# evapachetti/3d_vit_ensemble

Hardware: NVIDIA B200
Metric: ensemble volumes/sec (inference, fwd+bwd train) at 1/2/4/8 B200 vs CPU ref (higher is better)
Workload: dtype bf16

## Files before the change

3d_vit_ensemble_b200/csrc/api.cu:

```cuda
#include <stdarg.h>

#include "common.cuh"
#include "kernels.cuh"
#include "tc.cuh"

namespace vit3d {

static thread_local char g_err[512] = "";
static unsigned long long g_launches = 0;
void count_launch() { __atomic_fetch_add(&g_launches, 1ull, __ATOMIC_RELAXED); }

void set_error(const char* fmt, ...) {
  va_list ap;
  va_start(ap, fmt);
  vsnprintf(g_err, sizeof(g_err), fmt, ap);
  va_end(ap);
}
int cuda_fail(cudaError_t e, const char* what, const char* file, int line) {
  set_error("CUDA error %d (%s) at %s:%d: %s", (int)e, cudaGetErrorString(e), file, line, what);
  return VIT3D_ERR_CUDA;
}
int sm_count() {
  static thread_local int cached_dev = -1, cached = 0;
  int dev = 0;
  if (cudaGetDevice(&dev) != cudaSuccess) return 148;
  if (dev != cached_dev) {
    cudaDeviceProp p;
    if (cudaGetDeviceProperties(&p, dev) != cudaSuccess) return 148;
    cached = p.multiProcessorCount;
    cached_dev = dev;
  }
  return cached;
}

static int g_tuning[VIT3D_TUNE_COUNT] = {
    0,
    0,
    0,
    0,
    0,
    0,
    1,
    1,
    0,
    1,
    0,
    0,
    0,
    0,
    0,
};
constexpr unsigned kLiveTuningKeys =
    1u << VIT3D_TUNE_ATTN_THREADS | 1u << VIT3D_TUNE_MLP_PAIR | 1u << VIT3D_TUNE_WGRAD_RED | 1u << VIT3D_TUNE_ATTN_BWD |
    1u << VIT3D_TUNE_RES_PAIR | 1u << VIT3D_TUNE_ATTN_TF32 | 1u << VIT3D_TUNE_PATCH_TALL | 1u << VIT3D_TUNE_PATCH_CLUSTER |
    1u << VIT3D_TUNE_ATTN_FWD_UNIT;
static bool tuning_key_live(int key) { return key >= 0 && key < VIT3D_TUNE_COUNT && ((kLiveTuningKeys >> key) & 1u); }
int tuning(int key) {
  return (key >= 0 && key < VIT3D_TUNE_COUNT) ? __atomic_load_n(&g_tuning[key], __ATOMIC_RELAXED) : 0;
}

static inline int act_f32(int prec) { return prec != VIT3D_PREC_BF16; }

}

using namespace vit3d;

extern "C" {

int vit3d_version(void) { return VIT3D_VERSION; }
const char* vit3d_last_error(void) { return g_err; }

int vit3d_device_info(int* sms, int* cc) {
  int dev = 0;
  V3_CUDA(cudaGetDevice(&dev));
  cudaDeviceProp p;
  V3_CUDA(cudaGetDeviceProperties(&p, dev));
  if (sms) *sms = p.multiProcessorCount;
  if (cc) *cc = p.major * 10 + p.minor;
  return VIT3D_OK;
}
int vit3d_set_tuning(int key, int value) {
  V3_REQUIRE(tuning_key_live(key), "set_tuning: unknown or retired key %d", key);
  __atomic_store_n(&g_tuning[key], value, __ATOMIC_RELAXED);
  return VIT3D_OK;
}
int vit3d_get_tuning(int key) {
  V3_REQUIRE(tuning_key_live(key), "get_tuning: unknown or retired key %d", key);
  return tuning(key);
}
unsigned long long vit3d_launch_count(void) { return __atomic_load_n(&g_launches, __ATOMIC_RELAXED); }
int vit3d_act_bytes(int prec) { return prec == VIT3D_PREC_BF16 ? 2 : 4; }
int vit3d_tc_supported(int prec, int M, int N, int K) { return tc_linear_supported(prec, M, N, K) ? 1 : 0; }

int vit3d_patch_gather(const float* x, float* patches, int B, int X, int Y, int Z, int p0, int p1, int p2,
                       vit3d_stream_t stream) {
  V3_REQUIRE(B >= 0 && p0 > 0 && p1 > 0 && p2 > 0 && X >= p0 && Y >= p1 && Z >= p2, "patch_gather: bad shape");
  if (B == 0) return VIT3D_OK;
  V3_REQUIRE(x && patches, "patch_gather: null pointer");
  return launch_patch_gather(x, patches, 1, B, X, Y, Z, p0, p1, p2, as_stream(stream));
}

size_t vit3d_patch_embed_ws_bytes(int B, int X, int Y, int Z, int p0, int p1, int p2, int H, int prec) {
  (void)prec;
  const size_t P = (size_t)(X / p0) * (Y / p1) * (Z / p2);
  const size_t Kp = (size_t)p0 * p1 * p2;
  return sizeof(float) * ((size_t)B * P * Kp + (size_t)B * P * H) + 256;
}

int vit3d_patch_embed_fwd(const float* x, const float* w, const float* bias, const float* cls, const float* pos,
                          float* tokens, int B, int X, int Y, int Z, int p0, int p1, int p2, int H, int prec, void* ws,
                          size_t ws_bytes, vit3d_stream_t stream) {
  V3_REQUIRE(x && w && bias && cls && pos && tokens, "patch_embed_fwd: null pointer");
  V3_REQUIRE(B >= 0 && p0 > 0 && p1 > 0 && p2 > 0 && X >= p0 && Y >= p1 && Z >= p2 && H > 0, "patch_embed_fwd: bad shape");
  cudaStream_t st = as_stream(stream);
  const int P = (X / p0) * (Y / p1) * (Z / p2), Kp = p0 * p1 * p2, S = P + 1;
  if (B == 0) return VIT3D_OK;
  if (prec == VIT3D_PREC_BF16 && tc_patch_embed_supported(B, X, Y, Z, p0, p1, p2, H)) {
    int rc = tc_patch_embed_fwd(x, w, bias, pos, tokens, B, X, Y, Z, p0, p1, p2, H, st);
    if (rc != VIT3D_OK) return rc;
    return launch_cls_rows(cls, pos, tokens, B, S, H, st);
  }
  V3_REQUIRE(ws && ws_bytes >= vit3d_patch_embed_ws_bytes(B, X, Y, Z, p0, p1, p2, H, prec), "patch_embed_fwd: workspace too small");
  if (prec == VIT3D_PREC_TF32 && tc_patch_embed_supported(B, X, Y, Z, p0, p1, p2, H) &&
      (size_t)B * X * Y * Z * sizeof(float) <= ws_bytes) {
    float* xr = reinterpret_cast<float*>(ws);
    int rc = launch_round_tf32(x, xr, (long long)B * X * Y * Z, st);
    if (rc != VIT3D_OK) return rc;
    rc = tc_patch_embed_fwd(xr, w, bias, pos, tokens, B, X, Y, Z, p0, p1, p2, H, st);
    if (rc != VIT3D_OK) return rc;
    return launch_cls_rows(cls, pos, tokens, B, S, H, st);
  }
  float* patches = reinterpret_cast<float*>(ws);
  int rc = launch_patch_gather(x, patches, 1, B, X, Y, Z, p0, p1, p2, st);
  if (rc != VIT3D_OK) return rc;
  SgemmArgs g;
  g.A = patches; g.sa_m = Kp; g.sa_k = 1;
  g.B = w; g.sb_k = 1; g.sb_n = Kp;
  g.C = tokens; g.ldc = H;
  g.bias = bias; g.rowadd = pos; g.row_group = P;
  g.M = B * P; g.N = H; g.K = Kp;
  rc = launch_sgemm(g, st);
  if (rc != VIT3D_OK) return rc;
  return launch_cls_rows(cls, pos, tokens, B, S, H, st);
}

int vit3d_patch_embed_bwd(const float* x, const float* dtokens, float* dw, float* dbias, float* dcls, float* dpos, int B,
                          int X, int Y, int Z, int p0, int p1, int p2, int H, int prec, void* ws, size_t ws_bytes,
                          vit3d_stream_t stream) {
  V3_REQUIRE(x && dtokens && dw && dbias && dcls && dpos, "patch_embed_bwd: null pointer");
  V3_REQUIRE(ws && ws_bytes >= vit3d_patch_embed_ws_bytes(B, X, Y, Z, p0, p1, p2, H, prec), "patch_embed_bwd: workspace too small");
  cudaStream_t st = as_stream(stream);
  const int P = (X / p0) * (Y / p1) * (Z / p2), Kp = p0 * p1 * p2, S = P + 1;
  if (B == 0) return VIT3D_OK;
  int rc;
  if (prec == VIT3D_PREC_BF16 && tc_wgrad_supported(prec, B * P, H, Kp)) {
    __nv_bfloat16* patches = reinterpret_cast<__nv_bfloat16*>(ws);
    __nv_bfloat16* dYb = patches + (size_t)B * P * Kp;
    rc = launch_patch_gather(x, patches, 0, B, X, Y, Z, p0, p1, p2, st);
    if (rc != VIT3D_OK) return rc;
    rc = launch_gather_patch_rows(dtokens, dYb, 0, B, P, H, st);
    if (rc != VIT3D_OK) return rc;
    rc = tc_gemm_wgrad(dYb, patches, dw, H, Kp, B * P, st);
    if (rc != VIT3D_OK) return rc;
    rc = launch_colsum(dYb, 0, dbias, B * P, H, st);
    if (rc != VIT3D_OK) return rc;
    return launch_embed_param_grads(dtokens, dpos, dcls, B, S, H, st);
  }
  float* patches = reinterpret_cast<float*>(ws);
  float* dY = patches + (size_t)B * P * Kp;
  rc = launch_patch_gather(x, patches, 1, B, X, Y, Z, p0, p1, p2, st);
  if (rc != VIT3D_OK) return rc;
  rc = launch_gather_patch_rows(dtokens, dY, 1, B, P, H, st);
  if (rc != VIT3D_OK) return rc;
  SgemmArgs g;
  g.A = dY; g.sa_m = 1; g.sa_k = H;
  g.B = patches; g.sb_k = Kp; g.sb_n = 1;
  g.C = dw; g.ldc = Kp; g.accumulate = 1;
  g.M = H; g.N = Kp; g.K = B * P;
  g.splitk = pick_splitk(g.M, g.N, g.K);
  rc = launch_sgemm(g, st);
  if (rc != VIT3D_OK) return rc;
  rc = launch_colsum(dY, 1, dbias, B * P, H, st);
  if (rc != VIT3D_OK) return rc;
  return launch_embed_param_grads(dtokens, dpos, dcls, B, S, H, st);
}

int vit3d_patch_embed_dgrad(const float* dtokens, const float* w, const void* w_t_lp, float* dx, int B, int X, int Y, int Z,
                            int p0, int p1, int p2, int H, int prec, void* ws, size_t ws_bytes, vit3d_stream_t stream) {
  V3_REQUIRE(B >= 0 && p0 > 0 && p1 > 0 && p2 > 0 && X >= p0 && Y >= p1 && Z >= p2 && H > 0, "patch_embed_dgrad: bad shape");
  if (B == 0) return VIT3D_OK;
  V3_REQUIRE(dtokens && w && dx, "patch_embed_dgrad: null pointer");
  V3_REQUIRE(ws && ws_bytes >= vit3d_patch_embed_ws_bytes(B, X, Y, Z, p0, p1, p2, H, prec), "patch_embed_dgrad: workspace too small");
  cudaStream_t st = as_stream(stream);
  const int P = (X / p0) * (Y / p1) * (Z / p2), Kp = p0 * p1 * p2, S = P + 1;
  int rc;
  const bool aligned = ((reinterpret_cast<uintptr_t>(dtokens) | reinterpret_cast<uintptr_t>(dx) |
                         reinterpret_cast<uintptr_t>(w_t_lp)) & 15) == 0;
  if (prec != VIT3D_PREC_FP32 && w_t_lp && aligned && tc_patch_dgrad_supported(B, X, Y, Z, p0, p1, p2, H)) {
    const float* a = dtokens;
    if (prec == VIT3D_PREC_TF32) {
      V3_REQUIRE((size_t)B * S * H * sizeof(float) <= ws_bytes, "patch_embed_dgrad: workspace too small");
      float* dr = reinterpret_cast<float*>(ws);
      rc = launch_round_tf32(dtokens, dr, (long long)B * S * H, st);
      if (rc != VIT3D_OK) return rc;
      a = dr;
    }
    return tc_patch_dgrad(a, reinterpret_cast<const float*>(w_t_lp), dx, B, X, Y, Z, p0, p1, p2, H, st);
  }
  float* patches = reinterpret_cast<float*>(ws);
  float* dY = patches + (size_t)B * P * Kp;
  rc = launch_gather_patch_rows(dtokens, dY, 1, B, P, H, st);
  if (rc != VIT3D_OK) return rc;
  SgemmArgs g;
  g.A = dY; g.sa_m = H; g.sa_k = 1;
  g.B = w; g.sb_k = Kp; g.sb_n = 1;
  g.C = patches; g.ldc = Kp;
  g.M = B * P; g.N = Kp; g.K = H;
  rc = launch_sgemm(g, st);
  if (rc != VIT3D_OK) return rc;
  return launch_patch_scatter(patches, dx, B, X, Y, Z, p0, p1, p2, st);
}

int vit3d_ln_fwd(const float* x, const float* gamma, const float* beta, void* y, int y_bf16, float* mean, float* rstd,
                 int M, int H, float eps, vit3d_stream_t stream) {
  V3_REQUIRE(x && gamma && beta && y, "ln_fwd: null pointer");
  V3_REQUIRE(M >= 0 && H > 0, "ln_fwd: bad shape");
  return launch_ln_fwd(x, gamma, beta, y, y_bf16, mean, rstd, M, H, eps, as_stream(stream));
}
int vit3d_ln_bwd(const float* dy, const float* x, const float* mean, const float* rstd, const float* gamma,
                 const float* dres, float* dx, float* dgamma, float* dbeta, int M, int H, vit3d_stream_t stream) {
  V3_REQUIRE(dy && x && mean && rstd && gamma && dx && dgamma && dbeta, "ln_bwd: null pointer");
  V3_REQUIRE(M >= 0 && H > 0 && H <= 8192, "ln_bwd: bad shape");
  return launch_ln_bwd(dy, x, mean, rstd, gamma, dres, dx, dgamma, dbeta, M, H, as_stream(stream));
}

int vit3d_linear_fwd(const void* x, int ldx, int x_f32, const float* w, const void* w_lp, const float* bias,
                     const float* residual, void* y, int y_f32, void* pre, int act, int M, int N, int K, int prec,
                     vit3d_stream_t stream) {
  V3_REQUIRE(x && w && y, "linear_fwd: null pointer");
  V3_REQUIRE(M >= 0 && N > 0 && K > 0 && ldx >= K, "linear_fwd: bad shape M=%d N=%d K=%d ldx=%d", M, N, K, ldx);
  V3_REQUIRE(!(pre && residual), "linear_fwd: pre-activation output and residual are exclusive");
  cudaStream_t st = as_stream(stream);
  if (M == 0) return VIT3D_OK;
  const int xf = x_f32 || act_f32(prec);
  const int yf = y_f32 || residual != nullptr || act_f32(prec);
  if (prec != VIT3D_PREC_FP32 && tc_linear_supported(prec, M, N, K) && (prec == VIT3D_PREC_TF32 ? xf : !xf) &&
      (prec == VIT3D_PREC_TF32 || w_lp) && ldx == K) {
    TcLinear t;
    t.x = x; t.w = w_lp ? w_lp : (const void*)w; t.bias = bias; t.residual = residual;
    t.y = y; t.y_f32 = yf; t.pre = pre; t.act = act; t.M = M; t.N = N; t.K = K; t.prec = prec;
    return tc_linear_fwd(t, st);
  }
  if (N <= 8 && xf && yf && !residual && !pre && act == VIT3D_ACT_NONE)
    return launch_rowdot(reinterpret_cast<const float*>(x), ldx, w, bias, reinterpret_cast<float*>(y), M, N, K, st);
  SgemmArgs g;
  g.A = x; g.sa_m = ldx; g.sa_k = 1; g.a_f32 = xf;
  g.B = w; g.sb_k = 1; g.sb_n = K; g.b_f32 = 1;
  g.C = y; g.ldc = N; g.c_f32 = yf;
  g.bias = bias; g.residual = residual; g.ldr = N; g.pre = pre; g.act = act;
  g.M = M; g.N = N; g.K = K;
  return launch_sgemm(g, st);
}

int vit3d_linear_ln_supported(int M, int N, int K) { return tc_linear_ln_supported(VIT3D_PREC_BF16, M, N, K) ? 1 : 0; }

int vit3d_linear_ln_fwd(const void* x, const void* w_lp, const float* bias, const float* residual, float* y,
                        const float* gamma, const float* beta, float eps, void* ln_out, float* mean, float* rstd, int M,
                        int N, int K, vit3d_stream_t stream) {
  V3_REQUIRE(x && w_lp && y && gamma && beta && ln_out, "linear_ln_fwd: null pointer");
  V3_REQUIRE(M >= 0 && N > 0 && K > 0, "linear_ln_fwd: bad shape M=%d N=%d K=%d", M, N, K);
  if (M == 0) return VIT3D_OK;
  if (!tc_linear_ln_supported(VIT3D_PREC_BF16, M, N, K))
    V3_UNSUPPORTED("linear_ln_fwd: needs BF16 mode shapes with N == 256 (got M=%d N=%d K=%d)", M, N, K);
  TcLinear t;
  t.x = x; t.w = w_lp; t.bias = bias; t.residual = residual; t.y = y; t.y_f32 = 1; t.M = M; t.N = N; t.K = K;
  t.prec = VIT3D_PREC_BF16;
  t.ln_gamma = gamma; t.ln_beta = beta; t.ln_out = ln_out; t.ln_mean = mean; t.ln_rstd = rstd; t.ln_eps = eps;
  return tc_linear_fwd(t, as_stream(stream));
}

int vit3d_linear_bwd(const void* dy, int dy_f32, const void* x, int ldx, int x_f32, const float* w, const void* w_t_lp,
                     void* dx, int lddx, int dx_f32, float* dw, float* db, int M, int N, int K, int prec,
                     vit3d_stream_t stream) {
  V3_REQUIRE(dy && w, "linear_bwd: null pointer");
  V3_REQUIRE(M >= 0 && N > 0 && K > 0, "linear_bwd: bad shape");
  V3_REQUIRE(!dw || x, "linear_bwd: dw needs x");
  cudaStream_t st = as_stream(stream);
  if (M == 0) return VIT3D_OK;
  const int dyf = dy_f32 || act_f32(prec);
  const int xf = x_f32 || act_f32(prec);
  const int dxf = dx_f32 || act_f32(prec);
  int rc;
  if (dx) {
    if (prec == VIT3D_PREC_BF16 && !dyf && w_t_lp && (lddx <= 0 || lddx == K) && tc_linear_supported(prec, M, K, N)) {
      TcLinear t;
      t.x = dy; t.w = w_t_lp; t.y = dx; t.y_f32 = dxf; t.M = M; t.N = K; t.K = N; t.prec = prec;
      rc = tc_linear_fwd(t, st);
    } else {
      SgemmArgs g;
      g.A = dy; g.sa_m = N; g.sa_k = 1; g.a_f32 = dyf;
      g.B = w; g.sb_k = K; g.sb_n = 1; g.b_f32 = 1;
      g.C = dx; g.ldc = lddx > 0 ? lddx : K; g.c_f32 = dxf;
      g.M = M; g.N = K; g.K = N;
      rc = launch_sgemm(g, st);
    }
    if (rc != VIT3D_OK) return rc;
  }
  if (dw) {
    if (!dyf && !xf && ldx == K && tc_wgrad_supported(prec, M, N, K)) {
      rc = tc_gemm_wgrad(dy, x, dw, N, K, M, st);
    } else {
      SgemmArgs g;
      g.A = dy; g.sa_m = 1; g.sa_k = N; g.a_f32 = dyf;
      g.B = x; g.sb_k = ldx; g.sb_n = 1; g.b_f32 = xf;
      g.C = dw; g.ldc = K; g.c_f32 = 1; g.accumulate = 1;
      g.M = N; g.N = K; g.K = M;
      g.splitk = pick_splitk(g.M, g.N, g.K);
      rc = launch_sgemm(g, st);
    }
    if (rc != VIT3D_OK) return rc;
  }
  if (db) {
    rc = launch_colsum(dy, dyf, db, M, N, st);
    if (rc != VIT3D_OK) return rc;
  }
  return VIT3D_OK;
}

int vit3d_mlp_fwd(const void* xn, const void* w1_lp, const float* b1, const void* w2_lp, const float* b2,
                  const float* residual, float* out, int M, int H, int d, vit3d_stream_t stream) {
  V3_REQUIRE(xn && w1_lp && b1 && w2_lp && b2 && residual && out, "mlp_fwd: null pointer");
  V3_REQUIRE(M >= 0 && H > 0 && d > 0, "mlp_fwd: bad shape");
  if (M == 0) return VIT3D_OK;
  return tc_mlp2_fwd(xn, w1_lp, b1, w2_lp, b2, residual, out, nullptr, nullptr, 0.f, nullptr, 0, M, H, d, as_stream(stream));
}
int vit3d_mlp_supported(int M, int H, int d) { return tc_mlp2_supported(M, H, d) ? 1 : 0; }

int vit3d_mlp_ln_supported(int M, int H, int d) { return tc_mlp2_supported(M, H, d) ? 1 : 0; }
int vit3d_mlp_ln_fwd(const void* xn, const void* w1_lp, const float* b1, const void* w2_h, const float* b2,
                     const float* residual, float* out, const float* gamma, const float* beta, float eps, void* ln_out,
                     int M, int H, int d, vit3d_stream_t stream) {
  V3_REQUIRE(xn && w1_lp && b1 && w2_h && b2 && residual && out && gamma && beta && ln_out, "mlp_ln_fwd: null pointer");
  V3_REQUIRE(M >= 0 && H > 0 && d > 0, "mlp_ln_fwd: bad shape");
  if (M == 0) return VIT3D_OK;
  return tc_mlp2_fwd(xn, w1_lp, b1, w2_h, b2, residual, out, gamma, beta, eps, ln_out, 0, M, H, d, as_stream(stream));
}
int vit3d_mlp_lnf_fwd(const void* xn, const void* w1_lp, const float* b1, const void* w2_h, const float* b2,
                      const float* residual, const float* gamma, const float* beta, float eps, float* ln_out, int M, int H,
                      int d, vit3d_stream_t stream) {
  V3_REQUIRE(xn && w1_lp && b1 && w2_h && b2 && residual && gamma && beta && ln_out, "mlp_lnf_fwd: null pointer");
  V3_REQUIRE(M >= 0 && H > 0 && d > 0, "mlp_lnf_fwd: bad shape");
  if (M == 0) return VIT3D_OK;
  return tc_mlp2_fwd(xn, w1_lp, b1, w2_h, b2, residual, nullptr, gamma, beta, eps, ln_out, 1, M, H, d, as_stream(stream));
}

int vit3d_attn_fwd(const void* qkv, void* ctx, float* probs, int B, int S, int heads, int D, int prec,
                   vit3d_stream_t stream) {
  V3_REQUIRE(qkv && ctx, "attn_fwd: null pointer");
  V3_REQUIRE(B >= 0 && S > 0 && heads > 0 && D > 0, "attn_fwd: bad shape");
  cudaStream_t st = as_stream(stream);
  if (prec == VIT3D_PREC_BF16 && tc_attn_supported(S, heads, D)) return tc_attn_fwd(qkv, ctx, probs, S, B, S, heads, D, st);
  if (prec == VIT3D_PREC_TF32 && tc_attn_supported(S, heads, D) && tuning(VIT3D_TUNE_ATTN_TF32) != 0)
    return tc_attn_fwd_tf32(reinterpret_cast<const float*>(qkv), reinterpret_cast<float*>(ctx), probs, S, B, S, heads, D, 1, st);
  return launch_attn_fwd_generic(qkv, act_f32(prec), ctx, probs, B, S, heads, D, prec == VIT3D_PREC_TF32, st);
}
int vit3d_attn_fwd_padded(const void* qkv, void* ctx, float* probs, int probs_ld, int B, int S, int heads, int D,
                          vit3d_stream_t stream) {
  V3_REQUIRE(qkv && ctx && probs, "attn_fwd_padded: null pointer");
  V3_REQUIRE(B >= 0 && S > 0 && heads > 0 && D > 0 && probs_ld >= S, "attn_fwd_padded: bad shape");
  if (!tc_attn_supported(S, heads, D)) V3_UNSUPPORTED("attn_fwd_padded: unsupported shape S=%d heads=%d D=%d", S, heads, D);
  return tc_attn_fwd(qkv, ctx, probs, probs_ld, B, S, heads, D, as_stream(stream));
}
int vit3d_attn_padded_supported(int S, int heads, int D) { return tc_attn_supported(S, heads, D) ? 1 : 0; }
int vit3d_attn_bwd(const void* dctx, const void* qkv, void* dqkv, int B, int S, int heads, int D, int prec,
                   vit3d_stream_t stream) {
  V3_REQUIRE(dctx && qkv && dqkv, "attn_bwd: null pointer");
  V3_REQUIRE(B >= 0 && S > 0 && heads > 0 && D > 0, "attn_bwd: bad shape");
  if (prec == VIT3D_PREC_BF16 && tc_attn_supported(S, heads, D)) return tc_attn_bwd(dctx, qkv, dqkv, nullptr, nullptr, nullptr, B, S, heads, D, as_stream(stream));
  return launch_attn_bwd_generic(dctx, qkv, act_f32(prec), dqkv, B, S, heads, D, as_stream(stream));
}

int vit3d_gelu_fwd(const void* h, void* a, long long n, int prec, vit3d_stream_t stream) {
  V3_REQUIRE(h && a && n >= 0, "gelu_fwd: bad argument");
  return launch_gelu_fwd(h, a, n, act_f32(prec), as_stream(stream));
}
int vit3d_gelu_bwd(const void* da, const void* h, void* dh, long long n, int prec, vit3d_stream_t stream) {
  V3_REQUIRE(da && h && dh && n >= 0, "gelu_bwd: bad argument");
  return launch_gelu_bwd(da, h, dh, n, act_f32(prec), as_stream(stream));
}
int vit3d_gelu_dropout_bwd(const void* da, const void* h, void* dh, long long n, int prec, float p,
                           unsigned long long seed, unsigned site, unsigned step, const unsigned* step_dev,
                           vit3d_stream_t stream) {
  V3_REQUIRE(da && h && dh && n >= 0 && p >= 0.f && p < 1.f, "gelu_dropout_bwd: bad argument");
  if (!gelu_dropout_bwd_supported(da, h, dh, n, act_f32(prec)))
    V3_UNSUPPORTED("gelu_dropout_bwd: needs bf16 activations, 16-byte aligned buffers and n %% 8 == 0");
  return launch_gelu_dropout_bwd(da, h, dh, n, p, seed, site, step, step_dev, as_stream(stream));
}
int vit3d_dropout(const void* x, const void* residual, void* y, long long n, int is_f32, float p,
                  unsigned long long seed, unsigned site, unsigned step, const unsigned* step_dev,
                  vit3d_stream_t stream) {
  V3_REQUIRE(x && y && n >= 0 && p >= 0.f && p < 1.f, "dropout: bad argument");
  return launch_dropout(x, residual, y, n, is_f32, p, seed, site, step, step_dev, as_stream(stream));
}
int vit3d_dropout_mask(unsigned char* mask, long long n, float p, unsigned long long seed, unsigned site, unsigned step,
                       vit3d_stream_t stream) {
  V3_REQUIRE(mask && n >= 0 && p >= 0.f && p < 1.f, "dropout_mask: bad argument");
  return launch_dropout_mask(mask, n, p, seed, site, step, as_stream(stream));
}
int vit3d_dropout_masked(const void* x, const unsigned char* mask, const void* residual, void* y, long long n,
                         int is_f32, float p, vit3d_stream_t stream) {
  V3_REQUIRE(x && mask && y && n >= 0 && p >= 0.f && p < 1.f, "dropout_masked: bad argument");
  return launch_dropout_masked(x, mask, residual, y, n, is_f32, p, as_stream(stream));
}
int vit3d_cast_f32_to_bf16(const float* x, void* y, long long n, vit3d_stream_t stream) {
  V3_REQUIRE(x && y && n >= 0, "cast: bad argument");
  return launch_cast(x, 1, y, 0, n, as_stream(stream));
}
int vit3d_transpose_f32_to_bf16(const float* x, void* y, int rows, int cols, vit3d_stream_t stream) {
  V3_REQUIRE(x && y && rows >= 0 && cols >= 0, "transpose: bad argument");
  return launch_transpose_cast(x, y, rows, cols, as_stream(stream));
}
int vit3d_u8_to_f32(const unsigned char* x, float* y, long long n, float mean, vit3d_stream_t stream) {
  V3_REQUIRE(x && y && n >= 0, "u8_to_f32: bad argument");
  return launch_u8_to_f32(x, y, n, mean, as_stream(stream));
}
int vit3d_round_tf32(const float* x, float* y, long long n, vit3d_stream_t stream) {
  V3_REQUIRE(x && y && n >= 0, "round_tf32: bad argument");
  return launch_round_tf32(x, y, n, as_stream(stream));
}
int vit3d_cast_f32_to_f16(const float* x, void* y, long long n, vit3d_stream_t stream) {
// ... 170 lines not shown
```

3d_vit_ensemble_b200/csrc/tc.cuh:

```cuda
#pragma once
#include "common.cuh"

namespace vit3d {

struct TcLinear {
  const void* x = nullptr;
  const void* w = nullptr;
  const float* bias = nullptr;
  const float* residual = nullptr;
  void* y = nullptr;
  int y_f32 = 0;
  void* pre = nullptr;
  int act = 0;
  int M = 0, N = 0, K = 0, prec = 0;
  const float* ln_gamma = nullptr;
  const float* ln_beta = nullptr;
  void* ln_out = nullptr;
  float* ln_mean = nullptr;
  float* ln_rstd = nullptr;
  float ln_eps = 1e-6f;
  const uint32_t* drop_bits = nullptr;
  float drop_scale = 1.f;
  int store_dact = 0;
};
bool tc_linear_ln_supported(int prec, int M, int N, int K);
bool tc_res_supported(int M, int N, int K, bool ln);
int tc_gemm_res(const TcLinear& t, cudaStream_t st);

bool tc_linear_supported(int prec, int M, int N, int K);
int tc_linear_fwd(const TcLinear& t, cudaStream_t st);

bool tc_wgrad_supported(int prec, int M, int N, int K);
int tc_gemm_wgrad(const void* dy, const void* x, float* dw, int N, int K, int M, cudaStream_t st);
void tc_wgrad_plan(int N, int K, int M, int* bn, int* splits, int* tiles);
int tc_gemm_wgrad_partial(const void* dy, const void* x, float* ws, int N, int K, int M, cudaStream_t st);
int tc_gemm_wgrad_seg(const void* dy, const void* x, float* dw0, float* dw1, float* dw2, int seg_rows, int N, int K, int M,
                      cudaStream_t st);

bool tc_patch_embed_supported(int B, int X, int Y, int Z, int p0, int p1, int p2, int H);
int tc_patch_embed_fwd(const float* x, const float* w, const float* bias, const float* pos, float* tokens, int B, int X,
                       int Y, int Z, int p0, int p1, int p2, int H, cudaStream_t st);
bool tc_patch_dgrad_supported(int B, int X, int Y, int Z, int p0, int p1, int p2, int H);
int tc_patch_dgrad(const float* dtokens, const float* w_t, float* dx, int B, int X, int Y, int Z, int p0, int p1, int p2,
                   int H, cudaStream_t st);

bool tc_mlp3_supported(int M, int H, int d);
int tc_mlp3(const void* xn, const void* w1, const float* b1, const void* w2_h, const float* b2, const float* residual,
            float* y, const float* gamma, const float* beta, float eps, void* ln_out, int ln_f32, int M, int H, int d,
            cudaStream_t st);
bool tc_mlp2_supported(int M, int H, int d);
int tc_mlp2_fwd(const void* xn, const void* w1, const float* b1, const void* w2_h, const float* b2, const float* residual,
                float* y, const float* gamma, const float* beta, float eps, void* ln_out, int ln_f32, int M, int H, int d,
                cudaStream_t st);

bool tc_mlp_bwd_supported(int M, int H, int d);
int tc_mlp_bwd(const void* gy, const void* w2_t, const void* w1_t, const void* dact, void* dh, float* dxn, float* db1, int M,
               int H, int d, cudaStream_t st);

bool tc_attn_supported(int S, int heads, int D);
int tc_attn_fwd(const void* qkv, void* ctx, float* probs, int probs_ld, int B, int S, int heads, int D, cudaStream_t st);
int tc_attn_fwd_tf32(const float* qkv, float* ctx, float* probs, int probs_ld, int B, int S, int heads, int D, int round_out,
                     cudaStream_t st);
int tc_attn_bwd(const void* dctx, const void* qkv, void* dqkv, float* db_q, float* db_k, float* db_v, int B, int S,
                int heads, int D, cudaStream_t st);

}
```

include/vit3d.h:

```cpp
#ifndef VIT3D_H_
#define VIT3D_H_

#include <stddef.h>
#include <stdint.h>

#if defined(__GNUC__)
#pragma GCC visibility push(default)
#endif
#ifdef __cplusplus
extern "C" {
#endif

#define VIT3D_VERSION 100

typedef void* vit3d_stream_t;

enum { VIT3D_OK = 0, VIT3D_ERR_INVALID = -1, VIT3D_ERR_UNSUPPORTED = -2, VIT3D_ERR_CUDA = -3 };
enum { VIT3D_PREC_FP32 = 0, VIT3D_PREC_TF32 = 1, VIT3D_PREC_BF16 = 2 };
enum { VIT3D_ACT_NONE = 0, VIT3D_ACT_GELU = 1 };

int vit3d_version(void);
const char* vit3d_last_error(void);
int vit3d_device_info(int* sm_count, int* cc);
unsigned long long vit3d_launch_count(void);
enum { VIT3D_TUNE_ATTN_THREADS = 1, VIT3D_TUNE_MLP_PAIR = 5, VIT3D_TUNE_WGRAD_RED = 6, VIT3D_TUNE_ATTN_BWD = 7,
       VIT3D_TUNE_RES_PAIR = 8, VIT3D_TUNE_ATTN_TF32 = 9, VIT3D_TUNE_PATCH_TALL = 11, VIT3D_TUNE_PATCH_CLUSTER = 12,
       VIT3D_TUNE_ATTN_FWD_UNIT = 14, VIT3D_TUNE_COUNT = 15 };
int vit3d_set_tuning(int key, int value);
int vit3d_get_tuning(int key);
int vit3d_act_bytes(int prec);
int vit3d_tc_supported(int prec, int M, int N, int K);


int vit3d_patch_gather(const float* x, float* patches, int B, int X, int Y, int Z, int p0, int p1, int p2,
                       vit3d_stream_t stream);
size_t vit3d_patch_embed_ws_bytes(int B, int X, int Y, int Z, int p0, int p1, int p2, int H, int prec);
int vit3d_patch_embed_fwd(const float* x, const float* w, const float* bias, const float* cls, const float* pos,
                          float* tokens, int B, int X, int Y, int Z, int p0, int p1, int p2, int H, int prec,
                          void* ws, size_t ws_bytes, vit3d_stream_t stream);
int vit3d_patch_embed_bwd(const float* x, const float* dtokens, float* dw, float* dbias, float* dcls, float* dpos,
                          int B, int X, int Y, int Z, int p0, int p1, int p2, int H, int prec,
                          void* ws, size_t ws_bytes, vit3d_stream_t stream);
int vit3d_patch_embed_dgrad(const float* dtokens, const float* w, const void* w_t_lp, float* dx,
                            int B, int X, int Y, int Z, int p0, int p1, int p2, int H, int prec,
                            void* ws, size_t ws_bytes, vit3d_stream_t stream);

int vit3d_ln_fwd(const float* x, const float* gamma, const float* beta, void* y, int y_bf16, float* mean,
                 float* rstd, int M, int H, float eps, vit3d_stream_t stream);
int vit3d_ln_bwd(const float* dy, const float* x, const float* mean, const float* rstd, const float* gamma,
                 const float* dres, float* dx, float* dgamma, float* dbeta, int M, int H, vit3d_stream_t stream);

int vit3d_linear_fwd(const void* x, int ldx, int x_f32, const float* w, const void* w_lp, const float* bias,
                     const float* residual, void* y, int y_f32, void* pre, int act, int M, int N, int K, int prec,
                     vit3d_stream_t stream);
int vit3d_linear_ln_fwd(const void* x, const void* w_lp, const float* bias, const float* residual, float* y,
                        const float* gamma, const float* beta, float eps, void* ln_out, float* mean, float* rstd, int M,
                        int N, int K, vit3d_stream_t stream);
int vit3d_linear_ln_supported(int M, int N, int K);
int vit3d_linear_bwd(const void* dy, int dy_f32, const void* x, int ldx, int x_f32, const float* w, const void* w_t_lp,
                     void* dx, int lddx, int dx_f32, float* dw, float* db, int M, int N, int K, int prec,
                     vit3d_stream_t stream);

int vit3d_mlp_fwd(const void* xn, const void* w1_lp, const float* b1, const void* w2_h, const float* b2,
                  const float* residual, float* out, int M, int H, int d, vit3d_stream_t stream);
int vit3d_mlp_supported(int M, int H, int d);
int vit3d_mlp_ln_fwd(const void* xn, const void* w1_lp, const float* b1, const void* w2_h, const float* b2,
                     const float* residual, float* out, const float* gamma, const float* beta, float eps, void* ln_out,
                     int M, int H, int d, vit3d_stream_t stream);
int vit3d_mlp_ln_supported(int M, int H, int d);
int vit3d_mlp_lnf_fwd(const void* xn, const void* w1_lp, const float* b1, const void* w2_h, const float* b2,
                      const float* residual, const float* gamma, const float* beta, float eps, float* ln_out, int M, int H,
                      int d, vit3d_stream_t stream);

int vit3d_attn_fwd(const void* qkv, void* ctx, float* probs, int B, int S, int heads, int D, int prec,
                   vit3d_stream_t stream);
int vit3d_attn_fwd_padded(const void* qkv, void* ctx, float* probs, int probs_ld, int B, int S, int heads, int D,
                          vit3d_stream_t stream);
int vit3d_attn_padded_supported(int S, int heads, int D);
int vit3d_attn_bwd(const void* dctx, const void* qkv, void* dqkv, int B, int S, int heads, int D, int prec,
                   vit3d_stream_t stream);

int vit3d_gelu_fwd(const void* h, void* a, long long n, int prec, vit3d_stream_t stream);
int vit3d_gelu_bwd(const void* da, const void* h, void* dh, long long n, int prec, vit3d_stream_t stream);
int vit3d_gelu_dropout_bwd(const void* da, const void* h, void* dh, long long n, int prec, float p,
                           unsigned long long seed, unsigned site, unsigned step, const unsigned* step_dev,
                           vit3d_stream_t stream);
int vit3d_dropout(const void* x, const void* residual, void* y, long long n, int is_f32, float p,
                  unsigned long long seed, unsigned site, unsigned step, const unsigned* step_dev,
                  vit3d_stream_t stream);
int vit3d_dropout_mask(unsigned char* mask, long long n, float p, unsigned long long seed, unsigned site,
                       unsigned step, vit3d_stream_t stream);
int vit3d_dropout_masked(const void* x, const unsigned char* mask, const void* residual, void* y, long long n,
                         int is_f32, float p, vit3d_stream_t stream);
int vit3d_cast_f32_to_bf16(const float* x, void* y, long long n, vit3d_stream_t stream);
int vit3d_cast_bf16_to_f32(const void* x, float* y, long long n, vit3d_stream_t stream);
int vit3d_cast_f32_to_f16(const float* x, void* y, long long n, vit3d_stream_t stream);
int vit3d_u8_to_f32(const unsigned char* x, float* y, long long n, float mean, vit3d_stream_t stream);
int vit3d_transpose_f32_to_bf16(const float* x, void* y, int rows, int cols, vit3d_stream_t stream);
int vit3d_round_tf32(const float* x, float* y, long long n, vit3d_stream_t stream);
int vit3d_add_inplace(float* y, const float* x, long long n, vit3d_stream_t stream);

int vit3d_bce_logits_fwd(const float* logits, const float* labels, float pos_weight, const float* pos_weight_dev,
                         float* loss, int n, vit3d_stream_t stream);
int vit3d_bce_logits_bwd(const float* logits, const float* labels, float pos_weight, const float* pos_weight_dev,
                         const float* dloss, float* dlogits, int n, vit3d_stream_t stream);

int vit3d_meta_fwd(const float* feats, const float* w, const float* b, float* out, int B, int F, int C,
                   vit3d_stream_t stream);
int vit3d_meta_bwd(const float* dout, const float* out, const float* feats, const float* w, float* dfeats, float* dw,
                   float* db, int B, int F, int C, vit3d_stream_t stream);

int vit3d_sgd_step(float* p, const float* g, float* mom, long long n, float lr, float momentum, float weight_decay,
                   int first_step, float grad_scale, const float* lr_dev, vit3d_stream_t stream);
int vit3d_adam_step(float* p, const float* g, float* m, float* v, long long n, float lr, float beta1, float beta2,
                    float eps, float weight_decay, int step, float grad_scale, const float* lr_dev, const int* step_dev,
                    vit3d_stream_t stream);

#define VIT3D_MAX_DROP_SEGS 40
#define VIT3D_SHADOW_JOB_BYTES 40
#define VIT3D_SHADOW_TILE 64
int vit3d_memset_zero(void* p, size_t bytes, vit3d_stream_t stream);
int vit3d_train_supported(int B, int S, int H, int heads, int d);
int vit3d_dropout_bits(uint32_t* bits, int nseg, const unsigned* sites, const long long* nelems, float p,
                       unsigned long long seed, unsigned step, const unsigned* step_dev, vit3d_stream_t stream);
int vit3d_ln256_fwd(const float* x, const void* drop_bits, float drop_scale, float* x_dropped, const float* gamma,
                    const float* beta, void* y_bf16, float* y_f32, float* mean, float* rstd, int M, float eps,
                    vit3d_stream_t stream);
int vit3d_ln256_bwd(const float* dy, const float* x, const float* mean, const float* rstd, const float* gamma,
                    const float* dres, const void* drop_bits, float drop_scale, int mask_f32, float* dx, void* dx_bf16,
                    float* dgamma, float* dbeta, float* dbias, int M, vit3d_stream_t stream);
int vit3d_mul_colsum_bwd(const void* da, const void* dact, void* dh, float* db, int M, int d, vit3d_stream_t stream);
int vit3d_mlp_bwd(const void* gy, const void* w2_t_lp, const void* w1_t_lp, const void* dact, void* dh, float* dxn, float* db1,
                  int M, int H, int d, vit3d_stream_t stream);
int vit3d_mlp_bwd_supported(int M, int H, int d);
int vit3d_head_bwd(const float* dlogits, const float* encoded, const float* w, float* dencoded, float* dw, float* db, int B,
                   int S, int H, vit3d_stream_t stream);
int vit3d_refresh_shadows(const void* jobs, int njobs, int total_tiles, unsigned* step_dev, vit3d_stream_t stream);
int vit3d_fc1_train_fwd(const void* xn, const void* w1_lp, const float* b1, void* dact, void* act, const void* drop_bits,
                        float drop_scale, int M, int d, int H, vit3d_stream_t stream);
int vit3d_linear_res_train_fwd(const void* x, const void* w_lp, const float* bias, const float* residual, float* y,
                               const void* drop_bits, float drop_scale, const float* gamma, const float* beta, float eps,
                               void* ln_out, float* mean, float* rstd, int M, int N, int K, vit3d_stream_t stream);
int vit3d_wgrad(const void* dy, const void* x, float* dw0, float* dw1, float* dw2, int seg_rows, int M, int N, int K,
                vit3d_stream_t stream);
#define VIT3D_MAX_WGRAD_JOBS 48
#define VIT3D_WGRAD_JOB_BYTES 64
size_t vit3d_wgrad_ws_bytes(int M, int N, int K);
int vit3d_wgrad_partial(const void* dy, const void* x, float* ws, int M, int N, int K, int* bn, int* splits,
                        vit3d_stream_t stream);
int vit3d_wgrad_reduce(const void* host_jobs, int njobs, vit3d_stream_t stream);
int vit3d_attn_bwd_bias(const void* dctx, const void* qkv, void* dqkv, float* db_q, float* db_k, float* db_v, int B, int S,
                        int heads, int D, vit3d_stream_t stream);

#ifdef __cplusplus
}
#endif
#if defined(__GNUC__)
#pragma GCC visibility pop
#endif
#endif
```

Before: 627,200.

## Add warp-specialized persistent TMA/UMMA patch-embed kernel with cluster weight multicast

Adds a new persistent, warp-specialized patch-embedding GEMM for 256 filters. Separate TMA producer warps load input patches through a 5D tensor map and weights through a 3D map, with the weights multicast across a 2-CTA cluster. A single-thread UMMA issuer accumulates into double-buffered tensor memory, and 16 epilogue warps drain it. The cls-row write is folded into the kernel, which removes the separate cls launch and should let loads, MMAs and epilogue overlap across tiles. It is enabled by default when H=256 and there are enough tiles, so it adds new code paths, cluster-occupancy logic and an extra tuning key.

```diff
diff --git a/3d_vit_ensemble_b200/csrc/api.cu b/3d_vit_ensemble_b200/csrc/api.cu
--- a/3d_vit_ensemble_b200/csrc/api.cu
+++ b/3d_vit_ensemble_b200/csrc/api.cu
@@ -49,11 +49,12 @@
     0,
     0,
     0,
+    0,
 };
 constexpr unsigned kLiveTuningKeys =
     1u << VIT3D_TUNE_ATTN_THREADS | 1u << VIT3D_TUNE_MLP_PAIR | 1u << VIT3D_TUNE_WGRAD_RED | 1u << VIT3D_TUNE_ATTN_BWD |
     1u << VIT3D_TUNE_RES_PAIR | 1u << VIT3D_TUNE_ATTN_TF32 | 1u << VIT3D_TUNE_PATCH_TALL | 1u << VIT3D_TUNE_PATCH_CLUSTER |
-    1u << VIT3D_TUNE_ATTN_FWD_UNIT;
+    1u << VIT3D_TUNE_ATTN_FWD_UNIT | 1u << VIT3D_TUNE_PATCH_KERNEL;
 static bool tuning_key_live(int key) { return key >= 0 && key < VIT3D_TUNE_COUNT && ((kLiveTuningKeys >> key) & 1u); }
 int tuning(int key) {
   return (key >= 0 && key < VIT3D_TUNE_COUNT) ? __atomic_load_n(&g_tuning[key], __ATOMIC_RELAXED) : 0;
@@ -115,7 +116,10 @@
   cudaStream_t st = as_stream(stream);
   const int P = (X / p0) * (Y / p1) * (Z / p2), Kp = p0 * p1 * p2, S = P + 1;
   if (B == 0) return VIT3D_OK;
+  const bool stream256 = tuning(VIT3D_TUNE_PATCH_KERNEL) != 1 && tuning(VIT3D_TUNE_PATCH_TALL) == 0 &&
+                         tuning(VIT3D_TUNE_PATCH_CLUSTER) == 0 && tc_patch_embed256_supported(B, X, Y, Z, p0, p1, p2, H);
   if (prec == VIT3D_PREC_BF16 && tc_patch_embed_supported(B, X, Y, Z, p0, p1, p2, H)) {
+    if (stream256) return tc_patch_embed256_fwd(x, w, bias, cls, pos, tokens, B, X, Y, Z, p0, p1, p2, st);
     int rc = tc_patch_embed_fwd(x, w, bias, pos, tokens, B, X, Y, Z, p0, p1, p2, H, st);
     if (rc != VIT3D_OK) return rc;
     return launch_cls_rows(cls, pos, tokens, B, S, H, st);
@@ -126,6 +130,7 @@
     float* xr = reinterpret_cast<float*>(ws);
     int rc = launch_round_tf32(x, xr, (long long)B * X * Y * Z, st);
     if (rc != VIT3D_OK) return rc;
+    if (stream256) return tc_patch_embed256_fwd(xr, w, bias, cls, pos, tokens, B, X, Y, Z, p0, p1, p2, st);
     rc = tc_patch_embed_fwd(xr, w, bias, pos, tokens, B, X, Y, Z, p0, p1, p2, H, st);
     if (rc != VIT3D_OK) return rc;
     return launch_cls_rows(cls, pos, tokens, B, S, H, st);
diff --git a/3d_vit_ensemble_b200/csrc/k_tc_patch_embed.cu b/3d_vit_ensemble_b200/csrc/k_tc_patch_embed.cu
--- /dev/null
+++ b/3d_vit_ensemble_b200/csrc/k_tc_patch_embed.cu
@@ -0,0 +1,255 @@
+#include "ptx.cuh"
+#include "tc.cuh"
+#include "tc_epilogue.cuh"
+
+namespace vit3d {
+
+using namespace ptx;
+
+namespace {
+
+constexpr int PE_BM = 128, PE_BN = 256;
+constexpr int PE_A_BYTES = PE_BM * 128;
+constexpr int PE_B_BYTES = PE_BN * 128;
+constexpr int PE_EPI_WARPS = 16;
+constexpr int PE_THREADS = 96 + 32 * PE_EPI_WARPS;
+constexpr int PE_EPI_WARP_BYTES = 2048;
+
+template <int AST, int BST>
+struct PeCfg {
+  static constexpr int BAR_BYTES = (2 * AST + 2 * BST + 4) * 8 + 4;
+  static constexpr int SMEM_BYTES = AST * PE_A_BYTES + BST * PE_B_BYTES + PE_EPI_WARPS * PE_EPI_WARP_BYTES + 256;
+  static_assert(BAR_BYTES <= 256, "barriers overflow their shared-memory block");
+  static_assert(SMEM_BYTES <= 232448, "over the 227 KB shared-memory limit");
+};
+
+template <int AST, int BST>
+__global__ void __launch_bounds__(PE_THREADS, 1)
+tc_patch_embed_kernel(const __grid_constant__ CUtensorMap tmA, const __grid_constant__ CUtensorMap tmB, TcEpilogue ep,
+                      const float* __restrict__ cls, int B, int M, int tiles_m, int pblocks, int nkb, int tail_mmas) {
+  extern __shared__ __align__(1024) uint8_t smem_raw[];
+  uint8_t* aring = smem_raw;
+  if (smem_u32(aring) & 1023u) __trap();
+  uint8_t* bring = aring + AST * PE_A_BYTES;
+  uint8_t* epi_stage = bring + BST * PE_B_BYTES;
+  uint64_t* bars = reinterpret_cast<uint64_t*>(epi_stage + PE_EPI_WARPS * PE_EPI_WARP_BYTES);
+  uint64_t* a_full = bars;
+  uint64_t* a_empty = a_full + AST;
+  uint64_t* b_full = a_empty + AST;
+  uint64_t* b_empty = b_full + BST;
+  uint64_t* tmem_full = b_empty + BST;
+  uint64_t* tmem_empty = tmem_full + 2;
+  uint32_t* tmem_ptr_smem = reinterpret_cast<uint32_t*>(tmem_empty + 2);
+
+  const int warp = __shfl_sync(0xffffffffu, (int)(threadIdx.x >> 5), 0), lane = threadIdx.x & 31;
+  const int cl = ep.cluster;
+  const int vpt = ep.vols_per_tile;
+  if (warp == 0 && lane == 0) {
+    prefetch_tmap(&tmA);
+    prefetch_tmap(&tmB);
+    for (int s = 0; s < AST; ++s) {
+      mbar_init(&a_full[s], 1);
+      mbar_init(&a_empty[s], 1);
+    }
+    for (int s = 0; s < BST; ++s) {
+      mbar_init(&b_full[s], 1);
+      mbar_init(&b_empty[s], cl);
+    }
+    for (int b = 0; b < 2; ++b) {
+      mbar_init(&tmem_full[b], 1);
+      mbar_init(&tmem_empty[b], PE_EPI_WARPS);
+    }
+    fence_barrier_init();
+  }
+  if (warp == 1) tmem_alloc<2 * PE_BN>(tmem_ptr_smem);
+  tc_fence_before();
+  __syncthreads();
+  tc_fence_after();
+  const uint32_t tmem_base = *tmem_ptr_smem;
+  const uint32_t crank = cl > 1 ? cluster_ctarank() : 0u;
+  const uint16_t cmask = (uint16_t)((1u << cl) - 1u);
+  if (cl > 1) cluster_sync_all();
+  pdl_trigger();
+  pdl_wait();
+
+  if (warp == 0) {
+    if (lane == 0) {
+      int stage = 0;
+      uint32_t phase = 0;
+      for (int tm = blockIdx.x; tm < tiles_m; tm += gridDim.x)
+        for (int kb = 0; kb < nkb; ++kb) {
+          mbar_wait(&a_empty[stage], phase ^ 1);
+          mbar_arrive_expect_tx(&a_full[stage], PE_A_BYTES);
+          tma_load_5d(aring + stage * PE_A_BYTES, &tmA, &a_full[stage], (kb % pblocks) * 32, 0, kb / pblocks, 0, tm * vpt);
+          if (++stage == AST) { stage = 0; phase ^= 1; }
+        }
+    }
+    __syncwarp();
+  } else if (warp == 2) {
+    if (lane == 0) {
+      int stage = 0;
+      uint32_t phase = 0;
+      for (int tm = blockIdx.x; tm < tiles_m; tm += gridDim.x)
+        for (int kb = 0; kb < nkb; ++kb) {
+          mbar_wait(&b_empty[stage], phase ^ 1);
+          mbar_arrive_expect_tx(&b_full[stage], PE_B_BYTES);
+          uint8_t* dst = bring + stage * PE_B_BYTES + (int)crank * (PE_B_BYTES / cl);
+          const int c0 = (kb % pblocks) * 32, i = kb / pblocks, h0 = (int)crank * (PE_BN / cl);
+          if (cl > 1) tma_load_3d_mcast(dst, &tmB, &b_full[stage], c0, i, h0, cmask);
+          else tma_load_3d(dst, &tmB, &b_full[stage], c0, i, h0);
+          if (++stage == BST) { stage = 0; phase ^= 1; }
+        }
+    }
+    __syncwarp();
+  } else if (warp == 1) {
+    if (elect_one()) {
+      const uint32_t idesc = make_idesc(UMMA_FMT_TF32, PE_BM, PE_BN, 0, 0);
+      const uint64_t a_desc = make_smem_desc(smem_u32(aring), 16, 1024, UMMA_LAYOUT_SW128);
+      const uint64_t b_desc = make_smem_desc(smem_u32(bring), 16, 1024, UMMA_LAYOUT_SW128);
+      int as = 0, bs = 0, it = 0;
+      uint32_t aph = 0, bph = 0;
+      for (int tm = blockIdx.x; tm < tiles_m; tm += gridDim.x, ++it) {
+        const int buf = it & 1;
+        mbar_wait(&tmem_empty[buf], ((it >> 1) & 1) ^ 1);
+        tc_fence_after();
+        const uint32_t d_tmem = tmem_base + buf * PE_BN;
+        for (int kb = 0; kb < nkb; ++kb) {
+          mbar_wait(&a_full[as], aph);
+          mbar_wait(&b_full[bs], bph);
+          const uint64_t ad = a_desc + (uint64_t)((as * PE_A_BYTES) >> 4);
+          const uint64_t bd = b_desc + (uint64_t)((bs * PE_B_BYTES) >> 4);
+          const int nm = (kb % pblocks == pblocks - 1) ? tail_mmas : 4;
+#pragma unroll
+          for (int k = 0; k < 4; ++k)
+            if (k < nm) umma<true>(d_tmem, ad + 2 * k, bd + 2 * k, idesc, (kb > 0 || k > 0) ? 1u : 0u);
+          umma_commit(&a_empty[as]);
+          if (cl > 1) umma_commit_mcast(&b_empty[bs], cmask);
+          else umma_commit(&b_empty[bs]);
+          if (++as == AST) { as = 0; aph ^= 1; }
+          if (++bs == BST) { bs = 0; bph ^= 1; }
+        }
+        umma_commit(&tmem_full[buf]);
+      }
+    }
+    __syncwarp();
+  } else {
+    const int q = warp & 3;
+    const int part = (warp - 3) >> 2;
+    constexpr int CW = PE_BN / (PE_EPI_WARPS / 4);
+    const uint32_t stage = smem_u32(epi_stage + (warp - 3) * PE_EPI_WARP_BYTES);
+    const int S = ep.row_group + 1;
+    const int et = (int)threadIdx.x - 96;
+    int it = 0;
+    for (int tm = blockIdx.x; tm < tiles_m; tm += gridDim.x, ++it) {
+      const int buf = it & 1;
+      for (int e = et; e < vpt * PE_BN; e += PE_EPI_WARPS * 32) {
+        const int b = tm * vpt + e / PE_BN, h = e % PE_BN;
+        if (b < B) reinterpret_cast<float*>(ep.out)[(long long)b * S * PE_BN + h] = __ldg(cls + h) + __ldg(ep.rowadd + h);
+      }
+      mbar_wait(&tmem_full[buf], (it >> 1) & 1);
+      tc_fence_after();
+      const uint32_t taddr = tmem_base + ((uint32_t)(q * 32) << 16) + buf * PE_BN + part * CW;
+      epilogue_rows<CW, false, false>(ep, &tmA, &tmA, taddr, stage, lane, tm * PE_BM + q * 32, part * CW, M, PE_BN, ep.out,
+                                      0, 0);
+      tc_fence_before();
+      __syncwarp();
+      if (lane == 0) mbar_arrive(&tmem_empty[buf]);
+    }
+  }
+  tc_fence_before();
+  __syncthreads();
+  if (cl > 1) cluster_sync_all();
+  if (warp == 1) tmem_dealloc<2 * PE_BN>(tmem_base);
+}
+
+template <int AST, int BST>
+int launch_patch_embed(const CUtensorMap& ta, const CUtensorMap& tb, const TcEpilogue& ep, const float* cls, int B, int M,
+                       int tiles_m, int pblocks, int nkb, int tail_mmas, int grid, cudaStream_t st) {
+  auto kern = tc_patch_embed_kernel<AST, BST>;
+  static thread_local int configured_dev = -1;
+  int dev = 0;
+  V3_CUDA(cudaGetDevice(&dev));
+  if (configured_dev != dev) {
+    V3_CUDA(cudaFuncSetAttribute(kern, cudaFuncAttributeMaxDynamicSharedMemorySize, PeCfg<AST, BST>::SMEM_BYTES));
+    configured_dev = dev;
+  }
+  V3_CUDA(launch_pdl_cluster(kern, dim3(grid), dim3(PE_THREADS), (size_t)PeCfg<AST, BST>::SMEM_BYTES, st, ep.cluster, ta, tb,
+                             ep, cls, B, M, tiles_m, pblocks, nkb, tail_mmas));
+  V3_LAUNCH_CHECK();
+  return VIT3D_OK;
+}
+
+constexpr int PE_AST = 8, PE_BST = 2;
+
+int cluster_grid(int cl, int tiles_m) {
+  const int sms = sm_count();
+  static thread_local int cached_dev = -1, cached_cl = 0, nmax = 0;
+  int dev = 0;
+  if (cudaGetDevice(&dev) != cudaSuccess) return 0;
+  if (dev != cached_dev || cl != cached_cl) {
+    cached_dev = dev;
+    cached_cl = cl;
+    nmax = 0;
+    auto kern = tc_patch_embed_kernel<PE_AST, PE_BST>;
+    cudaFuncSetAttribute(kern, cudaFuncAttributeMaxDynamicSharedMemorySize, PeCfg<PE_AST, PE_BST>::SMEM_BYTES);
+    cudaLaunchConfig_t cfg = {};
+    cfg.gridDim = dim3(sms - sms % cl);
+    cfg.blockDim = dim3(PE_THREADS);
+    cfg.dynamicSmemBytes = PeCfg<PE_AST, PE_BST>::SMEM_BYTES;
+    cudaLaunchAttribute attr[1];
+    attr[0].id = cudaLaunchAttributeClusterDimension;
+    attr[0].val.clusterDim.x = cl; attr[0].val.clusterDim.y = 1; attr[0].val.clusterDim.z = 1;
+    cfg.attrs = attr;
+    cfg.numAttrs = 1;
+    if (cudaOccupancyMaxActiveClusters(&nmax, kern, &cfg) != cudaSuccess) { cudaGetLastError(); nmax = 0; }
+  }
+  int g = nmax * cl < sms ? nmax * cl : sms - sms % cl;
+  for (int tries = 0; tries < 8 && g >= cl; ++tries, g -= cl)
+    if ((tiles_m % g) % cl == 0) break;
+  return g >= cl && g * 10 >= sms * 9 && (tiles_m % g) % cl == 0 ? g : 0;
+}
+
+}
+
+bool tc_patch_embed256_supported(int B, int X, int Y, int Z, int p0, int p1, int p2, int H) {
+  if (H != PE_BN || !tc_patch_embed_supported(B, X, Y, Z, p0, p1, p2, H)) return false;
+  const int P = (X / p0) * (Y / p1);
+  return ceil_div((long long)B * P, PE_BM) >= sm_count();
+}
+
+int tc_patch_embed256_fwd(const float* x, const float* w, const float* bias, const float* cls, const float* pos,
+                          float* tokens, int B, int X, int Y, int Z, int p0, int p1, int p2, cudaStream_t st) {
+  if (!tc_patch_embed256_supported(B, X, Y, Z, p0, p1, p2, PE_BN)) V3_UNSUPPORTED("tc patch embedding (256 filters): unsupported geometry");
+  const int nx = X / p0, ny = Y / p1, P = nx * ny, inner = p1 * p2, vpt = PE_BM / P;
+  const int pblocks = ceil_div(inner, 32), nkb = p0 * pblocks;
+  const int tail_mmas = ceil_div(inner - 32 * (pblocks - 1), 8);
+  const int M = B * P, tiles_m = ceil_div(M, PE_BM);
+  const int ABL = tuning(VIT3D_TUNE_PATCH_KERNEL);
+  int cl = 2;
+  int grid = ABL == 2 ? 0 : cluster_grid(cl, tiles_m);
+  if (grid == 0) {
+    cl = 1;
+    grid = tiles_m < sm_count() ? tiles_m : sm_count();
+  }
+  CUtensorMap ta, tb;
+  {
+    cuuint64_t dims[5] = {(cuuint64_t)inner, (cuuint64_t)ny, (cuuint64_t)p0, (cuuint64_t)nx, (cuuint64_t)B};
+    cuuint64_t str[4] = {(cuuint64_t)inner * 4, (cuuint64_t)Y * Z * 4, (cuuint64_t)p0 * Y * Z * 4, (cuuint64_t)X * Y * Z * 4};
+    cuuint32_t box[5] = {32, (cuuint32_t)ny, 1, (cuuint32_t)nx, (cuuint32_t)vpt};
+    int rc = make_tmap_nd(&ta, x, 5, dims, str, box);
+    if (rc != VIT3D_OK) return rc;
+    cuuint64_t wd[3] = {(cuuint64_t)inner, (cuuint64_t)p0, (cuuint64_t)PE_BN};
+    cuuint64_t ws[2] = {(cuuint64_t)inner * 4, (cuuint64_t)p0 * inner * 4};
+    cuuint32_t wb[3] = {32, 1, (cuuint32_t)(PE_BN / cl)};
+    rc = make_tmap_nd(&tb, w, 3, wd, ws, wb);
+    if (rc != VIT3D_OK) return rc;
+  }
+  TcEpilogue ep;
+  ep.bias = bias; ep.rowadd = pos; ep.row_group = P; ep.out = tokens; ep.out_f32 = 1; ep.vols_per_tile = vpt;
+  ep.cluster = cl;
+  if (ABL == 3) return launch_patch_embed<4, 2>(ta, tb, ep, cls, B, M, tiles_m, pblocks, nkb, tail_mmas, grid, st);
+  if (ABL == 4) return launch_patch_embed<6, 3>(ta, tb, ep, cls, B, M, tiles_m, pblocks, nkb, tail_mmas, grid, st);
+  return launch_patch_embed<PE_AST, PE_BST>(ta, tb, ep, cls, B, M, tiles_m, pblocks, nkb, tail_mmas, grid, st);
+}
+
+}
diff --git a/3d_vit_ensemble_b200/csrc/tc.cuh b/3d_vit_ensemble_b200/csrc/tc.cuh
--- a/3d_vit_ensemble_b200/csrc/tc.cuh
+++ b/3d_vit_ensemble_b200/csrc/tc.cuh
@@ -40,6 +40,9 @@
 bool tc_patch_embed_supported(int B, int X, int Y, int Z, int p0, int p1, int p2, int H);
 int tc_patch_embed_fwd(const float* x, const float* w, const float* bias, const float* pos, float* tokens, int B, int X,
                        int Y, int Z, int p0, int p1, int p2, int H, cudaStream_t st);
+bool tc_patch_embed256_supported(int B, int X, int Y, int Z, int p0, int p1, int p2, int H);
+int tc_patch_embed256_fwd(const float* x, const float* w, const float* bias, const float* cls, const float* pos,
+                          float* tokens, int B, int X, int Y, int Z, int p0, int p1, int p2, cudaStream_t st);
 bool tc_patch_dgrad_supported(int B, int X, int Y, int Z, int p0, int p1, int p2, int H);
 int tc_patch_dgrad(const float* dtokens, const float* w_t, float* dx, int B, int X, int Y, int Z, int p0, int p1, int p2,
                    int H, cudaStream_t st);
diff --git a/include/vit3d.h b/include/vit3d.h
--- a/include/vit3d.h
+++ b/include/vit3d.h
@@ -25,7 +25,7 @@
 unsigned long long vit3d_launch_count(void);
 enum { VIT3D_TUNE_ATTN_THREADS = 1, VIT3D_TUNE_MLP_PAIR = 5, VIT3D_TUNE_WGRAD_RED = 6, VIT3D_TUNE_ATTN_BWD = 7,
        VIT3D_TUNE_RES_PAIR = 8, VIT3D_TUNE_ATTN_TF32 = 9, VIT3D_TUNE_PATCH_TALL = 11, VIT3D_TUNE_PATCH_CLUSTER = 12,
-       VIT3D_TUNE_ATTN_FWD_UNIT = 14, VIT3D_TUNE_COUNT = 15 };
+       VIT3D_TUNE_ATTN_FWD_UNIT = 14, VIT3D_TUNE_PATCH_KERNEL = 15, VIT3D_TUNE_COUNT = 16 };
 int vit3d_set_tuning(int key, int value);
 int vit3d_get_tuning(int key);
 int vit3d_act_bytes(int prec);
```

Result: slower. 602,700 (median of 6 runs) (-3.9%).
